# pixeli99/SVD_Xtend

Hardware: NVIDIA H100
Metric: SVD UNet train-step frames/sec @ 14x320x512 bf16 (higher is better)
Workload: dtype bf16

## Files before the change

### svd_xtend_b200/csrc/attention.cu

```cuda
#include "common.cuh"
#include "../../include/svd_xtend_b200.h"
#include "host_util.h"

namespace svdx {

constexpr int AT_THREADS = 288;
constexpr int AT_PRODUCER = 8;
constexpr int AT_CONSUMER_WARPS = 8;
constexpr int TILE_BYTES = 128 * 64 * 2;
constexpr float LOG2E = 1.4426950408889634f;

struct AttnKParams {
  CUtensorMap tq, tk, tv, tdo;
  int heads, S, G, RT, inner_groups, tiles, gshift, gmask;
  long long outer_stride, inner_stride, tok_stride;
  float scale;
  bf16* o; long long ldo;
  float* lse;
  float* delta;
  bf16* dq; long long lddq;
  bf16* dk; long long lddk;
  bf16* dv; long long lddv;
};

struct RowInfo {
  long long token;
  int g;
  bool valid;
};

SVDX_DEVINL RowInfo row_info(const AttnKParams& p, int r, int tile, int outer, int inner0) {
  RowInfo ri;
  const int t = tile * p.RT + (r >> p.gshift);
  ri.g = r & p.gmask;
  ri.valid = t < p.S;
  ri.token = (long long)outer * p.outer_stride + (long long)(inner0 + ri.g) * p.inner_stride + (long long)t * p.tok_stride;
  return ri;
}

SVDX_DEVINL float fast_exp2(float x) {
  float y;
  asm("ex2.approx.ftz.f32 %0, %1;" : "=f"(y) : "f"(x));
  return y;
}

SVDX_DEVINL void mma_abt64(float (&d)[32], uint32_t a_rows, uint32_t b_rows) {
  const uint64_t a = make_smem_desc_sw128(a_rows, 16, 1024), b = make_smem_desc_sw128(b_rows, 16, 1024);
  wgmma_fence();
#pragma unroll
  for (int ks = 0; ks < 4; ++ks) wgmma_ss_n64<0, 0>(d, a + 2 * ks, b + 2 * ks, ks > 0 ? 1u : 0u);
  wgmma_commit();
}
SVDX_DEVINL void mma_pb64(float (&acc)[32], const float (&p)[32], uint32_t b_rows) {
  const uint64_t b = make_smem_desc_sw128(b_rows, 8192, 1024);
  wgmma_fence();
#pragma unroll
  for (int ks = 0; ks < 4; ++ks)
    wgmma_rs_n64_tb(acc, pack_bf16x2(p[8 * ks], p[8 * ks + 1]), pack_bf16x2(p[8 * ks + 2], p[8 * ks + 3]),
                    pack_bf16x2(p[8 * ks + 4], p[8 * ks + 5]), pack_bf16x2(p[8 * ks + 6], p[8 * ks + 7]), b + (2048 >> 4) * ks, 1u);
  wgmma_commit();
}
SVDX_DEVINL int frag_col(int i, int lane) { return 8 * (i >> 2) + 2 * (lane & 3) + (i & 1); }
SVDX_DEVINL int frag_hi(int i) { return (i >> 1) & 1; }
SVDX_DEVINL float quad_max(float v) { return fmaxf(fmaxf(v, __shfl_xor_sync(0xffffffffu, v, 1)), __shfl_xor_sync(0xffffffffu, fmaxf(v, __shfl_xor_sync(0xffffffffu, v, 1)), 2)); }
SVDX_DEVINL float quad_sum(float v) { v += __shfl_xor_sync(0xffffffffu, v, 1); return v + __shfl_xor_sync(0xffffffffu, v, 2); }

SVDX_DEVINL void store_frag_rows(bf16* row_lo, bf16* row_hi, const float (&d)[32], float inv_lo, float inv_hi, int lane) {
#pragma unroll
  for (int j = 0; j < 8; ++j) {
    const int c = 8 * j + 2 * (lane & 3);
    if (row_lo) *reinterpret_cast<uint32_t*>(row_lo + c) = pack_bf16x2(d[4 * j] * inv_lo, d[4 * j + 1] * inv_lo);
    if (row_hi) *reinterpret_cast<uint32_t*>(row_hi + c) = pack_bf16x2(d[4 * j + 2] * inv_hi, d[4 * j + 3] * inv_hi);
  }
}

SVDX_DEVINL void decode_block(const AttnKParams& p, int& tile, int& head, int& outer, int& inner0) {
  tile = blockIdx.x;
  head = blockIdx.y;
  outer = blockIdx.z / p.inner_groups;
  inner0 = (blockIdx.z % p.inner_groups) * p.G;
}

SVDX_DEVINL void release(uint32_t bar, int lane) {
  __syncwarp();
  if (lane == 0) mbar_arrive(bar);
}

constexpr int FWD_KV_STAGES = 2;
constexpr int FWD_SMEM = 1024 + TILE_BYTES + FWD_KV_STAGES * 2 * TILE_BYTES + 256;

__global__ void __launch_bounds__(AT_THREADS, 1) attn_fwd_kernel(const __grid_constant__ AttnKParams p) {
  extern __shared__ uint8_t smem_raw[];
  const uint32_t base = (smem_u32(smem_raw) + 1023u) & ~1023u;
  const uint32_t sQ = base;
  const uint32_t sKV = sQ + TILE_BYTES;
  const uint32_t sBar = sKV + FWD_KV_STAGES * 2 * TILE_BYTES;
  const uint32_t b_qfull = sBar;
  const uint32_t b_kvfull = sBar + 8;
  const uint32_t b_kvempty = sBar + 8 * 3;

  const int warp = threadIdx.x >> 5, lane = threadIdx.x & 31;
  int tile, head, outer, inner0;
  decode_block(p, tile, head, outer, inner0);
  const int nkv = p.tiles;

  if (warp == AT_PRODUCER && lane == 0) {
    prefetch_tmap(&p.tq); prefetch_tmap(&p.tk); prefetch_tmap(&p.tv);
    mbar_init(b_qfull, 1);
    for (int i = 0; i < FWD_KV_STAGES; ++i) { mbar_init(b_kvfull + 8 * i, 1); mbar_init(b_kvempty + 8 * i, AT_CONSUMER_WARPS); }
    fence_barrier_init();
  }
  __syncthreads();

  if (warp == AT_PRODUCER) {
    if (lane == 0) {
      mbar_expect_tx(b_qfull, TILE_BYTES);
      tma_load_4d(&p.tq, b_qfull, sQ, head * 64, inner0, tile * p.RT, outer);
      for (int j = 0; j < nkv; ++j) {
        const int st = j % FWD_KV_STAGES;
        mbar_wait_mma(b_kvempty + 8 * st, ((j / FWD_KV_STAGES) & 1) ^ 1);
        mbar_expect_tx(b_kvfull + 8 * st, 2 * TILE_BYTES);
        tma_load_4d(&p.tk, b_kvfull + 8 * st, sKV + st * 2 * TILE_BYTES, head * 64, inner0, j * p.RT, outer);
        tma_load_4d(&p.tv, b_kvfull + 8 * st, sKV + st * 2 * TILE_BYTES + TILE_BYTES, head * 64, inner0, j * p.RT, outer);
      }
    }
    return;
  }
  const int wg = warp >> 2;
  const int r_lo = wg * 64 + (warp & 3) * 16 + (lane >> 2);
  const RowInfo ri[2] = {row_info(p, r_lo, tile, outer, inner0), row_info(p, r_lo + 8, tile, outer, inner0)};
  const float sc = p.scale * LOG2E;
  float m_run[2] = {-INFINITY, -INFINITY}, l_run[2] = {0.f, 0.f};
  float o[32];
#pragma unroll
  for (int i = 0; i < 32; ++i) o[i] = 0.f;
  mbar_wait_mma(b_qfull, 0);
  for (int j = 0; j < nkv; ++j) {
    const int st = j % FWD_KV_STAGES;
    const uint32_t sK = sKV + st * 2 * TILE_BYTES, sV = sK + TILE_BYTES;
    mbar_wait_mma(b_kvfull + 8 * st, (j / FWD_KV_STAGES) & 1);
    float s0[32], s1[32];
    mma_abt64(s0, sQ + wg * 8192, sK);
    mma_abt64(s1, sQ + wg * 8192, sK + 8192);
    wgmma_wait<0>();
    reg_fence(s0); reg_fence(s1);
    const int kvalid = p.S - j * p.RT;
    if (!(p.G == 1 && kvalid >= 128)) {
#pragma unroll
      for (int i = 0; i < 32; ++i) {
        const int c0 = frag_col(i, lane), c1 = 64 + c0;
        const RowInfo& r = ri[frag_hi(i)];
        if (!(((c0 & p.gmask) == r.g) && ((c0 >> p.gshift) < kvalid))) s0[i] = -INFINITY;
        if (!(((c1 & p.gmask) == r.g) && ((c1 >> p.gshift) < kvalid))) s1[i] = -INFINITY;
      }
    }
    float bm[2] = {-INFINITY, -INFINITY};
#pragma unroll
    for (int i = 0; i < 32; ++i) bm[frag_hi(i)] = fmaxf(bm[frag_hi(i)], fmaxf(s0[i], s1[i]));
    float msc[2], alpha[2];
#pragma unroll
    for (int h = 0; h < 2; ++h) {
      const float m_new = fmaxf(m_run[h], quad_max(bm[h]));
      const float m_use = m_new == -INFINITY ? 0.f : m_new;
      alpha[h] = fast_exp2((m_run[h] - m_use) * sc);
      m_run[h] = m_new;
      msc[h] = m_use * sc;
      l_run[h] *= alpha[h];
    }
#pragma unroll
    for (int i = 0; i < 32; ++i) {
      const int h = frag_hi(i);
      o[i] *= alpha[h];
      s0[i] = fast_exp2(fmaf(s0[i], sc, -msc[h]));
      s1[i] = fast_exp2(fmaf(s1[i], sc, -msc[h]));
      l_run[h] += s0[i] + s1[i];
    }
    mma_pb64(o, s0, sV);
    mma_pb64(o, s1, sV + 8192);
    wgmma_wait<0>();
    reg_fence(o);
    release(b_kvempty + 8 * st, lane);
  }
  bf16* rows[2];
  float inv[2];
#pragma unroll
  for (int h = 0; h < 2; ++h) {
    const float l = quad_sum(l_run[h]);
    const float m_use = m_run[h] == -INFINITY ? 0.f : m_run[h];
    inv[h] = 1.f / l;
    rows[h] = ri[h].valid ? p.o + ri[h].token * p.ldo + head * 64 : nullptr;
    if (ri[h].valid && p.lse && (lane & 3) == 0) p.lse[ri[h].token * p.heads + head] = m_use * p.scale + __logf(l);
  }
  store_frag_rows(rows[0], rows[1], o, inv[0], inv[1], lane);
}

constexpr int BWD_STAGES = 2;
constexpr int BDQ_SMEM = 1024 + 2 * TILE_BYTES + BWD_STAGES * 2 * TILE_BYTES + 256;

__global__ void __launch_bounds__(AT_THREADS, 1) attn_bwd_dq_kernel(const __grid_constant__ AttnKParams p) {
  extern __shared__ uint8_t smem_raw[];
  const uint32_t base = (smem_u32(smem_raw) + 1023u) & ~1023u;
  const uint32_t sQ = base, sDO = sQ + TILE_BYTES;
  const uint32_t sKV = sDO + TILE_BYTES;
  const uint32_t sBar = sKV + BWD_STAGES * 2 * TILE_BYTES;
  const uint32_t b_qfull = sBar;
  const uint32_t b_kvfull = sBar + 8;
  const uint32_t b_kvempty = sBar + 8 * 3;

  const int warp = threadIdx.x >> 5, lane = threadIdx.x & 31;
  int tile, head, outer, inner0;
  decode_block(p, tile, head, outer, inner0);
  const int nkv = p.tiles;

  if (warp == AT_PRODUCER && lane == 0) {
    prefetch_tmap(&p.tq); prefetch_tmap(&p.tk); prefetch_tmap(&p.tv); prefetch_tmap(&p.tdo);
    mbar_init(b_qfull, 1);
    for (int i = 0; i < BWD_STAGES; ++i) { mbar_init(b_kvfull + 8 * i, 1); mbar_init(b_kvempty + 8 * i, AT_CONSUMER_WARPS); }
    fence_barrier_init();
  }
  __syncthreads();

  if (warp == AT_PRODUCER) {
    if (lane == 0) {
      mbar_expect_tx(b_qfull, 2 * TILE_BYTES);
      tma_load_4d(&p.tq, b_qfull, sQ, head * 64, inner0, tile * p.RT, outer);
      tma_load_4d(&p.tdo, b_qfull, sDO, head * 64, inner0, tile * p.RT, outer);
      for (int j = 0; j < nkv; ++j) {
        const int st = j % BWD_STAGES;
        mbar_wait_mma(b_kvempty + 8 * st, ((j / BWD_STAGES) & 1) ^ 1);
        mbar_expect_tx(b_kvfull + 8 * st, 2 * TILE_BYTES);
        tma_load_4d(&p.tk, b_kvfull + 8 * st, sKV + st * 2 * TILE_BYTES, head * 64, inner0, j * p.RT, outer);
        tma_load_4d(&p.tv, b_kvfull + 8 * st, sKV + st * 2 * TILE_BYTES + TILE_BYTES, head * 64, inner0, j * p.RT, outer);
      }
    }
    return;
  }
  const int wg = warp >> 2;
  const int r_lo = wg * 64 + (warp & 3) * 16 + (lane >> 2);
  const RowInfo ri[2] = {row_info(p, r_lo, tile, outer, inner0), row_info(p, r_lo + 8, tile, outer, inner0)};
  const float sc = p.scale * LOG2E;
  float lse2[2], dlt[2];
#pragma unroll
  for (int h = 0; h < 2; ++h) {
    lse2[h] = ri[h].valid ? p.lse[ri[h].token * p.heads + head] * LOG2E : 0.f;
    dlt[h] = ri[h].valid ? p.delta[ri[h].token * p.heads + head] : 0.f;
  }
  float dq[32];
#pragma unroll
  for (int i = 0; i < 32; ++i) dq[i] = 0.f;
  mbar_wait_mma(b_qfull, 0);
  for (int j = 0; j < nkv; ++j) {
    const int st = j % BWD_STAGES;
    const uint32_t sK = sKV + st * 2 * TILE_BYTES, sV = sK + TILE_BYTES;
    mbar_wait_mma(b_kvfull + 8 * st, (j / BWD_STAGES) & 1);
    const int kvalid = p.S - j * p.RT;
    const bool nomask = (p.G == 1) && (kvalid >= 128);
#pragma unroll 1
    for (int kh = 0; kh < 2; ++kh) {
      float s[32], dp[32];
      mma_abt64(s, sQ + wg * 8192, sK + kh * 8192);
      mma_abt64(dp, sDO + wg * 8192, sV + kh * 8192);
      wgmma_wait<0>();
      reg_fence(s); reg_fence(dp);
#pragma unroll
      for (int i = 0; i < 32; ++i) {
        const int c = kh * 64 + frag_col(i, lane), h = frag_hi(i);
        const bool ok = ri[h].valid && (nomask || (((c & p.gmask) == ri[h].g) && ((c >> p.gshift) < kvalid)));
        const float pr = ok ? fast_exp2(fmaf(s[i], sc, -lse2[h])) * p.scale : 0.f;
        s[i] = pr * (dp[i] - dlt[h]);
      }
      mma_pb64(dq, s, sK + kh * 8192);
      wgmma_wait<0>();
      reg_fence(dq);
    }
    release(b_kvempty + 8 * st, lane);
  }
  store_frag_rows(ri[0].valid ? p.dq + ri[0].token * p.lddq + head * 64 : nullptr,
                  ri[1].valid ? p.dq + ri[1].token * p.lddq + head * 64 : nullptr, dq, 1.f, 1.f, lane);
}

constexpr int BKV_SMEM = 1024 + 2 * TILE_BYTES + BWD_STAGES * 2 * TILE_BYTES + 1024 + 256;

__global__ void __launch_bounds__(AT_THREADS, 1) attn_bwd_dkv_kernel(const __grid_constant__ AttnKParams p) {
  extern __shared__ uint8_t smem_raw[];
  const uint32_t base = (smem_u32(smem_raw) + 1023u) & ~1023u;
  const uint32_t sK = base, sV = sK + TILE_BYTES;
  const uint32_t sQD = sV + TILE_BYTES;
  const uint32_t sVec = sQD + BWD_STAGES * 2 * TILE_BYTES;
  const uint32_t sBar = sVec + 1024;
  const uint32_t b_kvfull = sBar;
  const uint32_t b_qfull = sBar + 8;
  const uint32_t b_qempty = sBar + 8 * 3;
  float* vec = reinterpret_cast<float*>(smem_raw + (sVec - smem_u32(smem_raw)));

  const int warp = threadIdx.x >> 5, lane = threadIdx.x & 31;
  int tile, head, outer, inner0;
  decode_block(p, tile, head, outer, inner0);
  const int nq = p.tiles;

  if (warp == AT_PRODUCER && lane == 0) {
    prefetch_tmap(&p.tq); prefetch_tmap(&p.tk); prefetch_tmap(&p.tv); prefetch_tmap(&p.tdo);
    mbar_init(b_kvfull, 1);
    for (int i = 0; i < BWD_STAGES; ++i) { mbar_init(b_qfull + 8 * i, 1); mbar_init(b_qempty + 8 * i, AT_CONSUMER_WARPS); }
    fence_barrier_init();
  }
  __syncthreads();

  if (warp == AT_PRODUCER) {
    if (lane == 0) {
      mbar_expect_tx(b_kvfull, 2 * TILE_BYTES);
      tma_load_4d(&p.tk, b_kvfull, sK, head * 64, inner0, tile * p.RT, outer);
      tma_load_4d(&p.tv, b_kvfull, sV, head * 64, inner0, tile * p.RT, outer);
      for (int i = 0; i < nq; ++i) {
        const int st = i % BWD_STAGES;
        mbar_wait_mma(b_qempty + 8 * st, ((i / BWD_STAGES) & 1) ^ 1);
        mbar_expect_tx(b_qfull + 8 * st, 2 * TILE_BYTES);
        tma_load_4d(&p.tq, b_qfull + 8 * st, sQD + st * 2 * TILE_BYTES, head * 64, inner0, i * p.RT, outer);
        tma_load_4d(&p.tdo, b_qfull + 8 * st, sQD + st * 2 * TILE_BYTES + TILE_BYTES, head * 64, inner0, i * p.RT, outer);
      }
    }
    return;
  }
  const int wg = warp >> 2;
  const int r_lo = wg * 64 + (warp & 3) * 16 + (lane >> 2);
  const RowInfo ki[2] = {row_info(p, r_lo, tile, outer, inner0), row_info(p, r_lo + 8, tile, outer, inner0)};
  const float sc = p.scale * LOG2E;
  const int vr = threadIdx.x & 127;
  auto load_stat = [&](int i) -> float {
    const RowInfo qi = row_info(p, vr, i, outer, inner0);
    if (threadIdx.x < 128) return qi.valid ? p.lse[qi.token * p.heads + head] * LOG2E : INFINITY;
    return qi.valid ? p.delta[qi.token * p.heads + head] : 0.f;
  };
  float stat = load_stat(0);
  float dv[32], dk[32];
#pragma unroll
  for (int i = 0; i < 32; ++i) { dv[i] = 0.f; dk[i] = 0.f; }
  mbar_wait_mma(b_kvfull, 0);
  for (int i = 0; i < nq; ++i) {
    named_bar_sync(1, 32 * AT_CONSUMER_WARPS);
    vec[threadIdx.x] = stat;
    named_bar_sync(1, 32 * AT_CONSUMER_WARPS);
    if (i + 1 < nq) stat = load_stat(i + 1);
    const int st = i % BWD_STAGES;
    const uint32_t sQ = sQD + st * 2 * TILE_BYTES, sDO = sQ + TILE_BYTES;
    mbar_wait_mma(b_qfull + 8 * st, (i / BWD_STAGES) & 1);
#pragma unroll 1
    for (int qh = 0; qh < 2; ++qh) {
      float s[32], dp[32];
      mma_abt64(s, sK + wg * 8192, sQ + qh * 8192);
      mma_abt64(dp, sV + wg * 8192, sDO + qh * 8192);
      wgmma_wait<0>();
      reg_fence(s); reg_fence(dp);
#pragma unroll
      for (int k = 0; k < 32; ++k) {
        const int c = qh * 64 + frag_col(k, lane);
        const RowInfo& r = ki[frag_hi(k)];
        const bool ok = r.valid && (p.G == 1 || (c & p.gmask) == r.g);
        const float pr = ok ? fast_exp2(fmaf(s[k], sc, -vec[c])) : 0.f;
        s[k] = pr;
        dp[k] = (pr * p.scale) * (dp[k] - vec[128 + c]);
      }
      mma_pb64(dv, s, sDO + qh * 8192);
      mma_pb64(dk, dp, sQ + qh * 8192);
      wgmma_wait<0>();
      reg_fence(dv); reg_fence(dk);
    }
    release(b_qempty + 8 * st, lane);
  }
  store_frag_rows(ki[0].valid ? p.dv + ki[0].token * p.lddv + head * 64 : nullptr,
                  ki[1].valid ? p.dv + ki[1].token * p.lddv + head * 64 : nullptr, dv, 1.f, 1.f, lane);
  store_frag_rows(ki[0].valid ? p.dk + ki[0].token * p.lddk + head * 64 : nullptr,
                  ki[1].valid ? p.dk + ki[1].token * p.lddk + head * 64 : nullptr, dk, 1.f, 1.f, lane);
}

__global__ void attn_delta_kernel(const bf16* __restrict__ o, long long ldo, const bf16* __restrict__ dout, long long lddo, long long tokens,
                                  int heads, float* __restrict__ delta) {
  const long long w = ((long long)blockIdx.x * blockDim.x + threadIdx.x) >> 5;
  const int lane = threadIdx.x & 31;
  if (w >= tokens * heads) return;
  const long long tok = w / heads;
  const int h = (int)(w - tok * heads);
  const float2 a = unpack_bf16x2(*reinterpret_cast<const uint32_t*>(o + tok * ldo + h * 64 + 2 * lane));
  const float2 b = unpack_bf16x2(*reinterpret_cast<const uint32_t*>(dout + tok * lddo + h * 64 + 2 * lane));
  const float s = warp_sum(a.x * b.x + a.y * b.y);
  if (lane == 0) delta[w] = s;
}

}

using namespace svdx;

static int attn_make_map(CUtensorMap* m, const void* ptr, int64_t ld, int cols, const SvdxAttn* d, int G, int RT) {
  const int outer = d->nseq / d->inner;
  uint64_t dims[4] = {(uint64_t)cols, (uint64_t)d->inner, (uint64_t)d->S, (uint64_t)outer};
  uint64_t strides[3] = {(uint64_t)(d->inner_stride * ld * 2), (uint64_t)(d->tok_stride * ld * 2), (uint64_t)(d->outer_stride * ld * 2)};
  if (d->inner == 1) strides[0] = (uint64_t)ld * 2;
  uint32_t box[4] = {64, (uint32_t)G, (uint32_t)RT, 1};
  return svdx_make_tmap(m, ptr, 4, dims, strides, box);
}

static int attn_setup(const SvdxAttn* d, AttnKParams& p, bool bwd, dim3& grid) {
  if (!d || !d->q || !d->k || !d->v) return svdx_fail(SVDX_E_BADARG, "attention: null pointer");
  if (d->heads <= 0 || d->S <= 0 || d->nseq <= 0 || d->inner <= 0 || d->nseq % d->inner) return svdx_fail(SVDX_E_BADARG, "attention: bad sequence geometry");
  if ((d->ldq % 8) || (d->ldk % 8) || (d->ldv % 8)) return svdx_fail(SVDX_E_BADARG, "attention: leading dims must be multiples of 8");
  memset(&p, 0, sizeof(p));
  int G = 1;
  if (d->inner > 1) {
    G = 1;
    while (G * 2 * d->S <= 128 && d->inner % (G * 2) == 0 && G < 64) G *= 2;
  }
  const int RT = 128 / G;
  if (d->inner > 1 && d->S > RT) return svdx_fail(SVDX_E_BADARG, "attention: strided sequences longer than 128 tokens are not supported");
  p.G = G; p.RT = RT; p.S = d->S; p.heads = d->heads;
  p.gmask = G - 1; p.gshift = 0;
  while ((1 << p.gshift) < G) ++p.gshift;
  p.inner_groups = d->inner / G;
  p.tiles = (d->S + RT - 1) / RT;
  p.outer_stride = d->outer_stride; p.inner_stride = d->inner_stride; p.tok_stride = d->tok_stride;
  p.scale = d->scale;
  const int cols = d->heads * 64;
  int rc;
  if ((rc = attn_make_map(&p.tq, d->q, d->ldq, cols, d, G, RT))) return rc;
  if ((rc = attn_make_map(&p.tk, d->k, d->ldk, cols, d, G, RT))) return rc;
  if ((rc = attn_make_map(&p.tv, d->v, d->ldv, cols, d, G, RT))) return rc;
  if (bwd) {
    if (!d->dout || !d->dq || !d->dk || !d->dv || !d->lse || !d->delta || !d->o) return svdx_fail(SVDX_E_BADARG, "attention_bwd: null pointer");
    if ((d->lddo % 8) || (d->lddq % 8) || (d->lddk % 8) || (d->lddv % 8) || (d->ldo % 8)) return svdx_fail(SVDX_E_BADARG, "attention_bwd: leading dims");
    if ((rc = attn_make_map(&p.tdo, d->dout, d->lddo, cols, d, G, RT))) return rc;
  } else {
    if (!d->o || (d->ldo % 8)) return svdx_fail(SVDX_E_BADARG, "attention_fwd: output");
  }
  p.o = reinterpret_cast<bf16*>(d->o); p.ldo = d->ldo;
  p.lse = d->lse; p.delta = d->delta;
  p.dq = reinterpret_cast<bf16*>(d->dq); p.lddq = d->lddq;
  p.dk = reinterpret_cast<bf16*>(d->dk); p.lddk = d->lddk;
  p.dv = reinterpret_cast<bf16*>(d->dv); p.lddv = d->lddv;
  const long long gz = (long long)(d->nseq / d->inner) * p.inner_groups;
  if (gz > 65535 || d->heads > 65535) return svdx_fail(SVDX_E_BADARG, "attention: grid too large");
  grid = dim3(p.tiles, d->heads, (unsigned)gz);
  return 0;
}

bool svdx_attention_small_eligible(const SvdxAttn* d);
int svdx_attention_small_fwd(const SvdxAttn* d, cudaStream_t st);
int svdx_attention_small_bwd(const SvdxAttn* d, cudaStream_t st);

extern "C" int svdx_attention_fwd(const SvdxAttn* d, void* stream_v) {
  cudaStream_t st = reinterpret_cast<cudaStream_t>(stream_v);
  if (svdx_attention_small_eligible(d)) return svdx_attention_small_fwd(d, st);
  AttnKParams p;
  dim3 grid;
// ... 6 lines not shown
    if (e != cudaSuccess) return svdx_fail_cuda(e, "attention_fwd: smem attribute");
    attr[slot] = true;
  }
  attn_fwd_kernel<<<grid, AT_THREADS, FWD_SMEM, st>>>(p);
  SVDX_CHECK_LAUNCH("attention_fwd");
  return SVDX_OK;
}

extern "C" int svdx_attention_bwd(const SvdxAttn* d, void* stream_v) {
  cudaStream_t st = reinterpret_cast<cudaStream_t>(stream_v);
  if (svdx_attention_small_eligible(d)) return svdx_attention_small_bwd(d, st);
  AttnKParams p;
  dim3 grid;
  int rc = attn_setup(d, p, true, grid);
  if (rc) return rc;
  static bool attr[SVDX_MAX_DEVICES] = {false};
  const int slot = svdx_device_slot();
  if (!attr[slot]) {
    cudaError_t e = cudaFuncSetAttribute(attn_bwd_dq_kernel, cudaFuncAttributeMaxDynamicSharedMemorySize, BDQ_SMEM);
    if (e == cudaSuccess) e = cudaFuncSetAttribute(attn_bwd_dkv_kernel, cudaFuncAttributeMaxDynamicSharedMemorySize, BKV_SMEM);
    if (e != cudaSuccess) return svdx_fail_cuda(e, "attention_bwd: smem attribute");
    attr[slot] = true;
  }
  const long long tokens = (long long)d->nseq * d->S;
  const long long warps = tokens * d->heads;
  attn_delta_kernel<<<(unsigned)((warps * 32 + 255) / 256), 256, 0, st>>>(reinterpret_cast<const bf16*>(d->o), d->ldo,
                                                                         reinterpret_cast<const bf16*>(d->dout), d->lddo, tokens, d->heads, d->delta);
  attn_bwd_dq_kernel<<<grid, AT_THREADS, BDQ_SMEM, st>>>(p);
  attn_bwd_dkv_kernel<<<grid, AT_THREADS, BKV_SMEM, st>>>(p);
  SVDX_CHECK_LAUNCH("attention_bwd");
  return SVDX_OK;
}
```

### svd_xtend_b200/csrc/common.cuh

```cuda
#pragma once
#include <cuda.h>
#include <cuda_bf16.h>
#include <cuda_runtime.h>
#include <stdint.h>
#include <stdio.h>

#include "wgmma.cuh"

namespace svdx {

typedef __nv_bfloat16 bf16;

#define SVDX_DEVINL __device__ __forceinline__

#ifndef SVDX_WAIT_TIMEOUT_CYCLES
#define SVDX_WAIT_TIMEOUT_CYCLES (4000000000ll)
#endif

SVDX_DEVINL uint32_t smem_u32(const void* p) { return (uint32_t)__cvta_generic_to_shared(p); }

SVDX_DEVINL uint32_t lane_id() { return threadIdx.x & 31; }

SVDX_DEVINL bool elect_one() {
  uint32_t pred = 0;
// ... 91 lines not shown
SVDX_DEVINL void tma_reduce_add_3d(const CUtensorMap* m, uint32_t src, int c0, int c1, int c2) {
  asm volatile("cp.reduce.async.bulk.tensor.3d.global.shared::cta.add.bulk_group [%0, {%2, %3, %4}], [%1];"
               ::"l"(reinterpret_cast<uint64_t>(m)), "r"(src), "r"(c0), "r"(c1), "r"(c2)
               : "memory");
}
SVDX_DEVINL void bulk_commit() { asm volatile("cp.async.bulk.commit_group;" ::: "memory"); }
template <int N>
SVDX_DEVINL void bulk_wait_read() { asm volatile("cp.async.bulk.wait_group.read %0;" ::"n"(N) : "memory"); }
template <int N>
SVDX_DEVINL void bulk_wait() { asm volatile("cp.async.bulk.wait_group %0;" ::"n"(N) : "memory"); }
SVDX_DEVINL void st_shared_v4(uint32_t addr, uint32_t a, uint32_t b, uint32_t c, uint32_t d) {
  asm volatile("st.shared.v4.b32 [%0], {%1, %2, %3, %4};" ::"r"(addr), "r"(a), "r"(b), "r"(c), "r"(d) : "memory");
}

SVDX_DEVINL void wgmma_fence() { asm volatile("wgmma.fence.sync.aligned;" ::: "memory"); }
SVDX_DEVINL void wgmma_commit() { asm volatile("wgmma.commit_group.sync.aligned;" ::: "memory"); }
template <int N>
SVDX_DEVINL void wgmma_wait() { asm volatile("wgmma.wait_group.sync.aligned %0;" ::"n"(N) : "memory"); }
template <int R>
SVDX_DEVINL void reg_fence(float (&d)[R]) {
#pragma unroll
  for (int i = 0; i < R; ++i) asm volatile("" : "+f"(d[i])::"memory");
}

SVDX_DEVINL void named_bar_sync(int id, int nthreads) { asm volatile("bar.sync %0, %1;" ::"r"(id), "r"(nthreads) : "memory"); }

SVDX_DEVINL uint64_t make_smem_desc_sw128(uint32_t saddr, uint32_t lbo_bytes, uint32_t sbo_bytes) {
  uint64_t d = 0;
  d |= (uint64_t)((saddr & 0x3FFFF) >> 4);
  d |= (uint64_t)((lbo_bytes >> 4) & 0x3FFF) << 16;
  d |= (uint64_t)((sbo_bytes >> 4) & 0x3FFF) << 32;
  d |= (uint64_t)1 << 62;
  return d;
}

SVDX_DEVINL float silu_f(float x) { return __fdividef(x, 1.0f + __expf(-x)); }
SVDX_DEVINL float silu_grad_f(float x) {
  const float s = __fdividef(1.0f, 1.0f + __expf(-x));
  return s * fmaf(x, 1.0f - s, 1.0f);
}
#define SVDX_HDINL __host__ __device__ __forceinline__
SVDX_HDINL float gelu_tail_log2(float ax) {
  float p = -1.92123457e-06f;
  p = fmaf(p, ax, 6.32884985e-05f);
  p = fmaf(p, ax, -0.000943420862f);
  p = fmaf(p, ax, 0.0085562719f);
  p = fmaf(p, ax, -0.0540522821f);
  p = fmaf(p, ax, -0.458381772f);
// ... 45 lines not shown
```

### svd_xtend_b200/raw.py

```python
from __future__ import annotations

import ctypes as C
import functools
import os
from typing import Optional, Sequence

import torch

from . import _lib
from ._lib import ACT_GELU, ACT_NONE, ACT_QUICK_GELU, A_CONV2D, A_ROWS, OUT_BF16, OUT_F32, OUT_F32_ATOMIC, SvdxAttn, SvdxTapGemm, load

bf16 = torch.bfloat16

_DTYPE_CODE = {torch.float32: 0, torch.bfloat16: 1, torch.float16: 2}


def dtype_code(t: torch.Tensor, what: str) -> int:
    try:
        return _DTYPE_CODE[t.dtype]
    except KeyError:
        raise TypeError(f"svd_xtend_b200: {what} has dtype {t.dtype}; supported: float32, bfloat16, float16") from None

LAUNCHES = [0]
_KERNELS_PER_CALL = {"svdx_groupnorm_apply_fused": 1, "svdx_attention_bwd": 3, "svdx_adamw_graph": 2, "svdx_adamw_p2p": 2,
                     "svdx_adamw_graph_ema": 2, "svdx_adamw_p2p_ema": 2, "svdx_ema_multi": 2, "svdx_adamw8bit": 2,
                     "svdx_adamw8bit_ema": 2}


def check(rc: int, what: str = "") -> None:
    LAUNCHES[0] += _KERNELS_PER_CALL.get(what, 1)
    _lib.check(rc, what)


ABLATE: set = set()
ACCOUNT = None
SHAPE_LOG = None


def _fam(family: str, flops: float = 0.0, nbytes: float = 0.0) -> bool:
    if ACCOUNT is not None:
        ACCOUNT(family, flops, nbytes)
    return family in ABLATE


def _stream() -> int:
    return torch.cuda.current_stream().cuda_stream

# ... 794 lines not shown
```

Before: 159.2.

## Software-pipeline attention kernels with ping-pong warpgroups, deeper stages, fused delta

The forward attention kernel now overlaps the next tile's QK^T wgmma with the previous tile's PV wgmma. It uses ping-pong named barriers so the two consumer warpgroups alternate tensor-core issue. The dq and dkv backward kernels are software-pipelined the same way by issuing the next half-tile's S/dP GEMMs while the current dS/P GEMMs run. Pipeline stages go from 2 to 4, and the separate delta kernel is folded into the dq kernel (the dkv producer reads lse/delta into per-stage smem). This costs more shared memory and register pressure, and adds an ordering dependency: the dkv kernel reads delta written by the dq kernel.

Result: faster. 161.3, median of 6 (+1.3%).

```diff
diff --git a/svd_xtend_b200/csrc/attention.cu b/svd_xtend_b200/csrc/attention.cu
--- a/svd_xtend_b200/csrc/attention.cu
+++ b/svd_xtend_b200/csrc/attention.cu
@@ -7,6 +7,7 @@
 constexpr int AT_THREADS = 288;
 constexpr int AT_PRODUCER = 8;
 constexpr int AT_CONSUMER_WARPS = 8;
+constexpr int AT_STAGES = 4;
 constexpr int TILE_BYTES = 128 * 64 * 2;
 constexpr float LOG2E = 1.4426950408889634f;
 
@@ -16,6 +17,7 @@
   long long outer_stride, inner_stride, tok_stride;
   float scale;
   bf16* o; long long ldo;
+  const bf16* dout; long long lddo;
   float* lse;
   float* delta;
   bf16* dq; long long lddq;
@@ -44,21 +46,33 @@
   return y;
 }
 
-SVDX_DEVINL void mma_abt64(float (&d)[32], uint32_t a_rows, uint32_t b_rows) {
+SVDX_DEVINL void mma_abt128(float (&d)[64], uint32_t a_rows, uint32_t b_rows) {
   const uint64_t a = make_smem_desc_sw128(a_rows, 16, 1024), b = make_smem_desc_sw128(b_rows, 16, 1024);
   wgmma_fence();
 #pragma unroll
-  for (int ks = 0; ks < 4; ++ks) wgmma_ss_n64<0, 0>(d, a + 2 * ks, b + 2 * ks, ks > 0 ? 1u : 0u);
+  for (int ks = 0; ks < 4; ++ks) wgmma_ss_n128<0, 0>(d, a + 2 * ks, b + 2 * ks, ks > 0 ? 1u : 0u);
   wgmma_commit();
 }
-SVDX_DEVINL void mma_pb64(float (&acc)[32], const float (&p)[32], uint32_t b_rows) {
+SVDX_DEVINL void mma_abt64x2(float (&s)[32], uint32_t a1, uint32_t b1, float (&dp)[32], uint32_t a2, uint32_t b2) {
+  const uint64_t da1 = make_smem_desc_sw128(a1, 16, 1024), db1 = make_smem_desc_sw128(b1, 16, 1024);
+  const uint64_t da2 = make_smem_desc_sw128(a2, 16, 1024), db2 = make_smem_desc_sw128(b2, 16, 1024);
+  wgmma_fence();
+#pragma unroll
+  for (int ks = 0; ks < 4; ++ks) wgmma_ss_n64<0, 0>(s, da1 + 2 * ks, db1 + 2 * ks, ks > 0 ? 1u : 0u);
+#pragma unroll
+  for (int ks = 0; ks < 4; ++ks) wgmma_ss_n64<0, 0>(dp, da2 + 2 * ks, db2 + 2 * ks, ks > 0 ? 1u : 0u);
+  wgmma_commit();
+}
+template <int KS>
+SVDX_DEVINL void mma_rb(float (&acc)[32], const uint32_t (&a)[4 * KS], uint32_t b_rows) {
   const uint64_t b = make_smem_desc_sw128(b_rows, 8192, 1024);
-  wgmma_fence();
-#pragma unroll
-  for (int ks = 0; ks < 4; ++ks)
-    wgmma_rs_n64_tb(acc, pack_bf16x2(p[8 * ks], p[8 * ks + 1]), pack_bf16x2(p[8 * ks + 2], p[8 * ks + 3]),
-                    pack_bf16x2(p[8 * ks + 4], p[8 * ks + 5]), pack_bf16x2(p[8 * ks + 6], p[8 * ks + 7]), b + (2048 >> 4) * ks, 1u);
-  wgmma_commit();
+#pragma unroll
+  for (int ks = 0; ks < KS; ++ks) wgmma_rs_n64_tb(acc, a[4 * ks], a[4 * ks + 1], a[4 * ks + 2], a[4 * ks + 3], b + (2048 >> 4) * ks, 1u);
+}
+template <int R>
+SVDX_DEVINL void pack_frag(uint32_t (&a)[R / 2], const float (&d)[R]) {
+#pragma unroll
+  for (int i = 0; i < R / 2; ++i) a[i] = pack_bf16x2(d[2 * i], d[2 * i + 1]);
 }
 SVDX_DEVINL int frag_col(int i, int lane) { return 8 * (i >> 2) + 2 * (lane & 3) + (i & 1); }
 SVDX_DEVINL int frag_hi(int i) { return (i >> 1) & 1; }
@@ -86,18 +100,56 @@
   if (lane == 0) mbar_arrive(bar);
 }
 
-constexpr int FWD_KV_STAGES = 2;
-constexpr int FWD_SMEM = 1024 + TILE_BYTES + FWD_KV_STAGES * 2 * TILE_BYTES + 256;
+struct PingPong {
+  int wg;
+  SVDX_DEVINL void start() const { if (wg == 1) named_bar_arrive(1, 32 * AT_CONSUMER_WARPS); }
+  SVDX_DEVINL void acquire() const { named_bar_sync(1 + wg, 32 * AT_CONSUMER_WARPS); }
+  SVDX_DEVINL void pass(bool last) const { if (wg == 0 || !last) named_bar_arrive(2 - wg, 32 * AT_CONSUMER_WARPS); }
+};
+
+constexpr int FWD_SMEM = 1024 + TILE_BYTES + AT_STAGES * 2 * TILE_BYTES + 256;
+
+SVDX_DEVINL void online_softmax(const AttnKParams& p, float (&s)[64], float (&m_run)[2], float (&l_run)[2], float (&alpha)[2],
+                                const RowInfo (&ri)[2], int kvalid, float sc, int lane) {
+  if (!(p.G == 1 && kvalid >= 128)) {
+#pragma unroll
+    for (int i = 0; i < 64; ++i) {
+      const int c = frag_col(i, lane);
+      const RowInfo& r = ri[frag_hi(i)];
+      if (!(((c & p.gmask) == r.g) && ((c >> p.gshift) < kvalid))) s[i] = -INFINITY;
+    }
+  }
+  float bm[2] = {-INFINITY, -INFINITY};
+#pragma unroll
+  for (int i = 0; i < 32; ++i) bm[frag_hi(i)] = fmaxf(bm[frag_hi(i)], fmaxf(s[i], s[i + 32]));
+  float msc[2];
+#pragma unroll
+  for (int h = 0; h < 2; ++h) {
+    const float m_new = fmaxf(m_run[h], quad_max(bm[h]));
+    const float m_use = m_new == -INFINITY ? 0.f : m_new;
+    alpha[h] = fast_exp2((m_run[h] - m_use) * sc);
+    m_run[h] = m_new;
+    msc[h] = m_use * sc;
+    l_run[h] *= alpha[h];
+  }
+#pragma unroll
+  for (int i = 0; i < 32; ++i) {
+    const int h = frag_hi(i);
+    s[i] = fast_exp2(fmaf(s[i], sc, -msc[h]));
+    s[i + 32] = fast_exp2(fmaf(s[i + 32], sc, -msc[h]));
+    l_run[h] += s[i] + s[i + 32];
+  }
+}
 
 __global__ void __launch_bounds__(AT_THREADS, 1) attn_fwd_kernel(const __grid_constant__ AttnKParams p) {
   extern __shared__ uint8_t smem_raw[];
   const uint32_t base = (smem_u32(smem_raw) + 1023u) & ~1023u;
   const uint32_t sQ = base;
   const uint32_t sKV = sQ + TILE_BYTES;
-  const uint32_t sBar = sKV + FWD_KV_STAGES * 2 * TILE_BYTES;
+  const uint32_t sBar = sKV + AT_STAGES * 2 * TILE_BYTES;
   const uint32_t b_qfull = sBar;
   const uint32_t b_kvfull = sBar + 8;
-  const uint32_t b_kvempty = sBar + 8 * 3;
+  const uint32_t b_kvempty = sBar + 8 * (1 + AT_STAGES);
 
   const int warp = threadIdx.x >> 5, lane = threadIdx.x & 31;
   int tile, head, outer, inner0;
@@ -107,7 +159,7 @@
   if (warp == AT_PRODUCER && lane == 0) {
     prefetch_tmap(&p.tq); prefetch_tmap(&p.tk); prefetch_tmap(&p.tv);
     mbar_init(b_qfull, 1);
-    for (int i = 0; i < FWD_KV_STAGES; ++i) { mbar_init(b_kvfull + 8 * i, 1); mbar_init(b_kvempty + 8 * i, AT_CONSUMER_WARPS); }
+    for (int i = 0; i < AT_STAGES; ++i) { mbar_init(b_kvfull + 8 * i, 1); mbar_init(b_kvempty + 8 * i, AT_CONSUMER_WARPS); }
     fence_barrier_init();
   }
   __syncthreads();
@@ -117,8 +169,8 @@
       mbar_expect_tx(b_qfull, TILE_BYTES);
       tma_load_4d(&p.tq, b_qfull, sQ, head * 64, inner0, tile * p.RT, outer);
       for (int j = 0; j < nkv; ++j) {
-        const int st = j % FWD_KV_STAGES;
-        mbar_wait_mma(b_kvempty + 8 * st, ((j / FWD_KV_STAGES) & 1) ^ 1);
+        const int st = j % AT_STAGES;
+        mbar_wait_mma(b_kvempty + 8 * st, ((j / AT_STAGES) & 1) ^ 1);
         mbar_expect_tx(b_kvfull + 8 * st, 2 * TILE_BYTES);
         tma_load_4d(&p.tk, b_kvfull + 8 * st, sKV + st * 2 * TILE_BYTES, head * 64, inner0, j * p.RT, outer);
         tma_load_4d(&p.tv, b_kvfull + 8 * st, sKV + st * 2 * TILE_BYTES + TILE_BYTES, head * 64, inner0, j * p.RT, outer);
@@ -130,57 +182,49 @@
   const int r_lo = wg * 64 + (warp & 3) * 16 + (lane >> 2);
   const RowInfo ri[2] = {row_info(p, r_lo, tile, outer, inner0), row_info(p, r_lo + 8, tile, outer, inner0)};
   const float sc = p.scale * LOG2E;
-  float m_run[2] = {-INFINITY, -INFINITY}, l_run[2] = {0.f, 0.f};
-  float o[32];
+  const uint32_t sQw = sQ + wg * 8192;
+  const PingPong pp{wg};
+  float m_run[2] = {-INFINITY, -INFINITY}, l_run[2] = {0.f, 0.f}, alpha[2];
+  float o[32], s[64];
+  uint32_t pa[32];
 #pragma unroll
   for (int i = 0; i < 32; ++i) o[i] = 0.f;
+  pp.start();
   mbar_wait_mma(b_qfull, 0);
-  for (int j = 0; j < nkv; ++j) {
-    const int st = j % FWD_KV_STAGES;
-    const uint32_t sK = sKV + st * 2 * TILE_BYTES, sV = sK + TILE_BYTES;
-    mbar_wait_mma(b_kvfull + 8 * st, (j / FWD_KV_STAGES) & 1);
-    float s0[32], s1[32];
-    mma_abt64(s0, sQ + wg * 8192, sK);
-    mma_abt64(s1, sQ + wg * 8192, sK + 8192);
+  mbar_wait_mma(b_kvfull, 0);
+  pp.acquire();
+  mma_abt128(s, sQw, sKV);
+  pp.pass(false);
+  wgmma_wait<0>();
+  reg_fence(s);
+  online_softmax(p, s, m_run, l_run, alpha, ri, p.S, sc, lane);
+  pack_frag<64>(pa, s);
+  for (int j = 1; j < nkv; ++j) {
+    const int st = j % AT_STAGES, pst = (j - 1) % AT_STAGES;
+    mbar_wait_mma(b_kvfull + 8 * st, (j / AT_STAGES) & 1);
+    pp.acquire();
+    mma_abt128(s, sQw, sKV + st * 2 * TILE_BYTES);
+    wgmma_fence();
+    mma_rb<8>(o, pa, sKV + pst * 2 * TILE_BYTES + TILE_BYTES);
+    wgmma_commit();
+    pp.pass(false);
+    wgmma_wait<1>();
+    reg_fence(s);
+    online_softmax(p, s, m_run, l_run, alpha, ri, p.S - j * p.RT, sc, lane);
     wgmma_wait<0>();
-    reg_fence(s0); reg_fence(s1);
-    const int kvalid = p.S - j * p.RT;
-    if (!(p.G == 1 && kvalid >= 128)) {
-#pragma unroll
-      for (int i = 0; i < 32; ++i) {
-        const int c0 = frag_col(i, lane), c1 = 64 + c0;
-        const RowInfo& r = ri[frag_hi(i)];
-        if (!(((c0 & p.gmask) == r.g) && ((c0 >> p.gshift) < kvalid))) s0[i] = -INFINITY;
-        if (!(((c1 & p.gmask) == r.g) && ((c1 >> p.gshift) < kvalid))) s1[i] = -INFINITY;
-      }
-    }
-    float bm[2] = {-INFINITY, -INFINITY};
-#pragma unroll
-    for (int i = 0; i < 32; ++i) bm[frag_hi(i)] = fmaxf(bm[frag_hi(i)], fmaxf(s0[i], s1[i]));
-    float msc[2], alpha[2];
-#pragma unroll
-    for (int h = 0; h < 2; ++h) {
-      const float m_new = fmaxf(m_run[h], quad_max(bm[h]));
-      const float m_use = m_new == -INFINITY ? 0.f : m_new;
-      alpha[h] = fast_exp2((m_run[h] - m_use) * sc);
-      m_run[h] = m_new;
-      msc[h] = m_use * sc;
-      l_run[h] *= alpha[h];
-    }
-#pragma unroll
-    for (int i = 0; i < 32; ++i) {
-      const int h = frag_hi(i);
-      o[i] *= alpha[h];
-      s0[i] = fast_exp2(fmaf(s0[i], sc, -msc[h]));
-      s1[i] = fast_exp2(fmaf(s1[i], sc, -msc[h]));
-      l_run[h] += s0[i] + s1[i];
-    }
-    mma_pb64(o, s0, sV);
-    mma_pb64(o, s1, sV + 8192);
-    wgmma_wait<0>();
-    reg_fence(o);
-    release(b_kvempty + 8 * st, lane);
-  }
+    reg_fence(o); reg_fence(pa);
+    release(b_kvempty + 8 * pst, lane);
+#pragma unroll
+    for (int i = 0; i < 32; ++i) o[i] *= alpha[frag_hi(i)];
+    pack_frag<64>(pa, s);
+  }
+  pp.acquire();
+  wgmma_fence();
+  mma_rb<8>(o, pa, sKV + ((nkv - 1) % AT_STAGES) * 2 * TILE_BYTES + TILE_BYTES);
+  wgmma_commit();
+  pp.pass(true);
+  wgmma_wait<0>();
+  reg_fence(o);
   bf16* rows[2];
   float inv[2];
 #pragma unroll
@@ -194,18 +238,35 @@
   store_frag_rows(rows[0], rows[1], o, inv[0], inv[1], lane);
 }
 
-constexpr int BWD_STAGES = 2;
-constexpr int BDQ_SMEM = 1024 + 2 * TILE_BYTES + BWD_STAGES * 2 * TILE_BYTES + 256;
+constexpr int BDQ_SMEM = 1024 + 2 * TILE_BYTES + AT_STAGES * 2 * TILE_BYTES + 256;
+
+SVDX_DEVINL float row_delta(const bf16* o, const bf16* dout, bool valid, int lane) {
+  const int q = lane & 3;
+  float t[8];
+#pragma unroll
+  for (int m = 0; m < 8; ++m) {
+    float2 a = make_float2(0.f, 0.f), b = a;
+    if (valid) {
+      a = unpack_bf16x2(*reinterpret_cast<const uint32_t*>(o + 2 * (q + 4 * m)));
+      b = unpack_bf16x2(*reinterpret_cast<const uint32_t*>(dout + 2 * (q + 4 * m)));
+    }
+    t[m] = fmaf(a.x, b.x, a.y * b.y);
+  }
+  const float w0 = t[0] + t[4], w1 = t[1] + t[5], w2 = t[2] + t[6], w3 = t[3] + t[7];
+  float v = (w0 + w2) + (w1 + w3);
+  v += __shfl_xor_sync(0xffffffffu, v, 2);
+  return v + __shfl_xor_sync(0xffffffffu, v, 1);
+}
 
 __global__ void __launch_bounds__(AT_THREADS, 1) attn_bwd_dq_kernel(const __grid_constant__ AttnKParams p) {
   extern __shared__ uint8_t smem_raw[];
   const uint32_t base = (smem_u32(smem_raw) + 1023u) & ~1023u;
   const uint32_t sQ = base, sDO = sQ + TILE_BYTES;
   const uint32_t sKV = sDO + TILE_BYTES;
-  const uint32_t sBar = sKV + BWD_STAGES * 2 * TILE_BYTES;
+  const uint32_t sBar = sKV + AT_STAGES * 2 * TILE_BYTES;
   const uint32_t b_qfull = sBar;
   const uint32_t b_kvfull = sBar + 8;
-  const uint32_t b_kvempty = sBar + 8 * 3;
+  const uint32_t b_kvempty = sBar + 8 * (1 + AT_STAGES);
 
   const int warp = threadIdx.x >> 5, lane = threadIdx.x & 31;
   int tile, head, outer, inner0;
@@ -215,7 +276,7 @@
   if (warp == AT_PRODUCER && lane == 0) {
     prefetch_tmap(&p.tq); prefetch_tmap(&p.tk); prefetch_tmap(&p.tv); prefetch_tmap(&p.tdo);
     mbar_init(b_qfull, 1);
-    for (int i = 0; i < BWD_STAGES; ++i) { mbar_init(b_kvfull + 8 * i, 1); mbar_init(b_kvempty + 8 * i, AT_CONSUMER_WARPS); }
+    for (int i = 0; i < AT_STAGES; ++i) { mbar_init(b_kvfull + 8 * i, 1); mbar_init(b_kvempty + 8 * i, AT_CONSUMER_WARPS); }
     fence_barrier_init();
   }
   __syncthreads();
@@ -226,8 +287,8 @@
       tma_load_4d(&p.tq, b_qfull, sQ, head * 64, inner0, tile * p.RT, outer);
       tma_load_4d(&p.tdo, b_qfull, sDO, head * 64, inner0, tile * p.RT, outer);
       for (int j = 0; j < nkv; ++j) {
-        const int st = j % BWD_STAGES;
-        mbar_wait_mma(b_kvempty + 8 * st, ((j / BWD_STAGES) & 1) ^ 1);
+        const int st = j % AT_STAGES;
+        mbar_wait_mma(b_kvempty + 8 * st, ((j / AT_STAGES) & 1) ^ 1);
         mbar_expect_tx(b_kvfull + 8 * st, 2 * TILE_BYTES);
         tma_load_4d(&p.tk, b_kvfull + 8 * st, sKV + st * 2 * TILE_BYTES, head * 64, inner0, j * p.RT, outer);
         tma_load_4d(&p.tv, b_kvfull + 8 * st, sKV + st * 2 * TILE_BYTES + TILE_BYTES, head * 64, inner0, j * p.RT, outer);
@@ -243,54 +304,68 @@
 #pragma unroll
   for (int h = 0; h < 2; ++h) {
     lse2[h] = ri[h].valid ? p.lse[ri[h].token * p.heads + head] * LOG2E : 0.f;
-    dlt[h] = ri[h].valid ? p.delta[ri[h].token * p.heads + head] : 0.f;
-  }
-  float dq[32];
+    dlt[h] = row_delta(p.o + ri[h].token * p.ldo + head * 64, p.dout + ri[h].token * p.lddo + head * 64, ri[h].valid, lane);
+    if (ri[h].valid && (lane & 3) == 0) p.delta[ri[h].token * p.heads + head] = dlt[h];
+  }
+  const uint32_t sQw = sQ + wg * 8192, sDOw = sDO + wg * 8192;
+  float dq[32], s[32], dp[32];
+  uint32_t ds[16];
 #pragma unroll
   for (int i = 0; i < 32; ++i) dq[i] = 0.f;
+  reg_fence(dq);
+  const int nu = 2 * nkv;
   mbar_wait_mma(b_qfull, 0);
-  for (int j = 0; j < nkv; ++j) {
-    const int st = j % BWD_STAGES;
-    const uint32_t sK = sKV + st * 2 * TILE_BYTES, sV = sK + TILE_BYTES;
-    mbar_wait_mma(b_kvfull + 8 * st, (j / BWD_STAGES) & 1);
+  mbar_wait_mma(b_kvfull, 0);
+  mma_abt64x2(s, sQw, sKV, dp, sDOw, sKV + TILE_BYTES);
+  for (int u = 0; u < nu; ++u) {
+    const int j = u >> 1, kh = u & 1, st = j % AT_STAGES;
+    const uint32_t sK = sKV + st * 2 * TILE_BYTES;
+    wgmma_wait<0>();
+    reg_fence(s); reg_fence(dp); reg_fence(dq); reg_fence(ds);
+    if (u >= 2 && kh == 0) release(b_kvempty + 8 * ((j - 1) % AT_STAGES), lane);
     const int kvalid = p.S - j * p.RT;
     const bool nomask = (p.G == 1) && (kvalid >= 128);
-#pragma unroll 1
-    for (int kh = 0; kh < 2; ++kh) {
-      float s[32], dp[32];
-      mma_abt64(s, sQ + wg * 8192, sK + kh * 8192);
-      mma_abt64(dp, sDO + wg * 8192, sV + kh * 8192);
-      wgmma_wait<0>();
-      reg_fence(s); reg_fence(dp);
-#pragma unroll
-      for (int i = 0; i < 32; ++i) {
-        const int c = kh * 64 + frag_col(i, lane), h = frag_hi(i);
+#pragma unroll
+    for (int i = 0; i < 32; i += 2) {
+      float v[2];
+#pragma unroll
+      for (int e = 0; e < 2; ++e) {
+        const int c = kh * 64 + frag_col(i + e, lane), h = frag_hi(i + e);
         const bool ok = ri[h].valid && (nomask || (((c & p.gmask) == ri[h].g) && ((c >> p.gshift) < kvalid)));
-        const float pr = ok ? fast_exp2(fmaf(s[i], sc, -lse2[h])) * p.scale : 0.f;
-        s[i] = pr * (dp[i] - dlt[h]);
+        const float pr = ok ? fast_exp2(fmaf(s[i + e], sc, -lse2[h])) * p.scale : 0.f;
+        v[e] = pr * (dp[i + e] - dlt[h]);
       }
-      mma_pb64(dq, s, sK + kh * 8192);
-      wgmma_wait<0>();
-      reg_fence(dq);
-    }
-    release(b_kvempty + 8 * st, lane);
-  }
+      ds[i / 2] = pack_bf16x2(v[0], v[1]);
+    }
+    const bool more = u + 1 < nu;
+    const int j1 = (u + 1) >> 1, st1 = j1 % AT_STAGES;
+    if (more && kh == 1) mbar_wait_mma(b_kvfull + 8 * st1, (j1 / AT_STAGES) & 1);
+    wgmma_fence();
+    mma_rb<4>(dq, ds, sK + kh * 8192);
+    wgmma_commit();
+    if (more) {
+      const uint32_t sK1 = sKV + st1 * 2 * TILE_BYTES, c1 = ((u + 1) & 1) * 8192;
+      mma_abt64x2(s, sQw, sK1 + c1, dp, sDOw, sK1 + TILE_BYTES + c1);
+    }
+  }
+  wgmma_wait<0>();
+  reg_fence(dq);
   store_frag_rows(ri[0].valid ? p.dq + ri[0].token * p.lddq + head * 64 : nullptr,
                   ri[1].valid ? p.dq + ri[1].token * p.lddq + head * 64 : nullptr, dq, 1.f, 1.f, lane);
 }
 
-constexpr int BKV_SMEM = 1024 + 2 * TILE_BYTES + BWD_STAGES * 2 * TILE_BYTES + 1024 + 256;
+constexpr int BKV_SMEM = 1024 + 2 * TILE_BYTES + AT_STAGES * 2 * TILE_BYTES + AT_STAGES * 1024 + 256;
 
 __global__ void __launch_bounds__(AT_THREADS, 1) attn_bwd_dkv_kernel(const __grid_constant__ AttnKParams p) {
   extern __shared__ uint8_t smem_raw[];
   const uint32_t base = (smem_u32(smem_raw) + 1023u) & ~1023u;
   const uint32_t sK = base, sV = sK + TILE_BYTES;
   const uint32_t sQD = sV + TILE_BYTES;
-  const uint32_t sVec = sQD + BWD_STAGES * 2 * TILE_BYTES;
-  const uint32_t sBar = sVec + 1024;
+  const uint32_t sVec = sQD + AT_STAGES * 2 * TILE_BYTES;
+  const uint32_t sBar = sVec + AT_STAGES * 1024;
   const uint32_t b_kvfull = sBar;
   const uint32_t b_qfull = sBar + 8;
-  const uint32_t b_qempty = sBar + 8 * 3;
+  const uint32_t b_qempty = sBar + 8 * (1 + AT_STAGES);
   float* vec = reinterpret_cast<float*>(smem_raw + (sVec - smem_u32(smem_raw)));
 
   const int warp = threadIdx.x >> 5, lane = threadIdx.x & 31;
@@ -301,89 +376,102 @@
   if (warp == AT_PRODUCER && lane == 0) {
     prefetch_tmap(&p.tq); prefetch_tmap(&p.tk); prefetch_tmap(&p.tv); prefetch_tmap(&p.tdo);
     mbar_init(b_kvfull, 1);
-    for (int i = 0; i < BWD_STAGES; ++i) { mbar_init(b_qfull + 8 * i, 1); mbar_init(b_qempty + 8 * i, AT_CONSUMER_WARPS); }
+    for (int i = 0; i < AT_STAGES; ++i) { mbar_init(b_qfull + 8 * i, 1 + 32); mbar_init(b_qempty + 8 * i, AT_CONSUMER_WARPS); }
     fence_barrier_init();
   }
   __syncthreads();
 
   if (warp == AT_PRODUCER) {
-    if (lane == 0) {
-      mbar_expect_tx(b_kvfull, 2 * TILE_BYTES);
-      tma_load_4d(&p.tk, b_kvfull, sK, head * 64, inner0, tile * p.RT, outer);
-      tma_load_4d(&p.tv, b_kvfull, sV, head * 64, inner0, tile * p.RT, outer);
+    {
+      if (lane == 0) {
+        mbar_expect_tx(b_kvfull, 2 * TILE_BYTES);
+        tma_load_4d(&p.tk, b_kvfull, sK, head * 64, inner0, tile * p.RT, outer);
+        tma_load_4d(&p.tv, b_kvfull, sV, head * 64, inner0, tile * p.RT, outer);
+      }
       for (int i = 0; i < nq; ++i) {
-        const int st = i % BWD_STAGES;
-        mbar_wait_mma(b_qempty + 8 * st, ((i / BWD_STAGES) & 1) ^ 1);
-        mbar_expect_tx(b_qfull + 8 * st, 2 * TILE_BYTES);
-        tma_load_4d(&p.tq, b_qfull + 8 * st, sQD + st * 2 * TILE_BYTES, head * 64, inner0, i * p.RT, outer);
-        tma_load_4d(&p.tdo, b_qfull + 8 * st, sQD + st * 2 * TILE_BYTES + TILE_BYTES, head * 64, inner0, i * p.RT, outer);
+        const int st = i % AT_STAGES;
+        mbar_wait_mma(b_qempty + 8 * st, ((i / AT_STAGES) & 1) ^ 1);
+        if (lane == 0) {
+          mbar_expect_tx(b_qfull + 8 * st, 2 * TILE_BYTES);
+          tma_load_4d(&p.tq, b_qfull + 8 * st, sQD + st * 2 * TILE_BYTES, head * 64, inner0, i * p.RT, outer);
+          tma_load_4d(&p.tdo, b_qfull + 8 * st, sQD + st * 2 * TILE_BYTES + TILE_BYTES, head * 64, inner0, i * p.RT, outer);
+        }
+#pragma unroll
+        for (int k = 0; k < 4; ++k) {
+          const int r = lane + 32 * k;
+          const RowInfo qi = row_info(p, r, i, outer, inner0);
+          vec[st * 256 + r] = qi.valid ? p.lse[qi.token * p.heads + head] * LOG2E : INFINITY;
+          vec[st * 256 + 128 + r] = qi.valid ? p.delta[qi.token * p.heads + head] : 0.f;
+        }
+        mbar_arrive(b_qfull + 8 * st);
       }
     }
     return;
   }
   const int wg = warp >> 2;
   const int r_lo = wg * 64 + (warp & 3) * 16 + (lane >> 2);
+  bool kval[2];
+  int kg[2];
+#pragma unroll
+  for (int h = 0; h < 2; ++h) {
+    const RowInfo r = row_info(p, r_lo + 8 * h, tile, outer, inner0);
+    kval[h] = r.valid;
+    kg[h] = r.g;
+  }
+  const float sc = p.scale * LOG2E;
+  const uint32_t sKw = sK + wg * 8192, sVw = sV + wg * 8192;
+  float dv[32], dk[32], s[32], dp[32];
+  uint32_t pt[16], dst[16];
+#pragma unroll
+  for (int i = 0; i < 32; ++i) { dv[i] = 0.f; dk[i] = 0.f; }
+  reg_fence(dv); reg_fence(dk);
+  const int nu = 2 * nq;
+  mbar_wait_mma(b_kvfull, 0);
+  mbar_wait_mma(b_qfull, 0);
+  mma_abt64x2(s, sKw, sQD, dp, sVw, sQD + TILE_BYTES);
+  for (int u = 0; u < nu; ++u) {
+    const int i = u >> 1, qh = u & 1, st = i % AT_STAGES;
+    const uint32_t sQ = sQD + st * 2 * TILE_BYTES, sDO = sQ + TILE_BYTES;
+    const float* lse2 = vec + st * 256 + qh * 64 + 2 * (lane & 3);
+    const float* dlt = lse2 + 128;
+    wgmma_wait<0>();
+    reg_fence(s); reg_fence(dp); reg_fence(dv); reg_fence(dk); reg_fence(pt); reg_fence(dst);
+    if (u >= 2 && qh == 0) release(b_qempty + 8 * ((i - 1) % AT_STAGES), lane);
+#pragma unroll
+    for (int k = 0; k < 32; k += 2) {
+      const float2 l2 = *reinterpret_cast<const float2*>(lse2 + 8 * (k >> 2));
+      const float2 d2 = *reinterpret_cast<const float2*>(dlt + 8 * (k >> 2));
+      float pr[2], ds[2];
+#pragma unroll
+      for (int e = 0; e < 2; ++e) {
+        const int c = qh * 64 + frag_col(k + e, lane);
+        const int h = frag_hi(k + e);
+        const bool ok = kval[h] && (p.G == 1 || (c & p.gmask) == kg[h]);
+        pr[e] = ok ? fast_exp2(fmaf(s[k + e], sc, -(e ? l2.y : l2.x))) : 0.f;
+        ds[e] = (pr[e] * p.scale) * (dp[k + e] - (e ? d2.y : d2.x));
+      }
+      pt[k / 2] = pack_bf16x2(pr[0], pr[1]);
+      dst[k / 2] = pack_bf16x2(ds[0], ds[1]);
+    }
+    const bool more = u + 1 < nu;
+    const int i1 = (u + 1) >> 1, st1 = i1 % AT_STAGES;
+    if (more && qh == 1) mbar_wait_mma(b_qfull + 8 * st1, (i1 / AT_STAGES) & 1);
+    wgmma_fence();
+    mma_rb<4>(dv, pt, sDO + qh * 8192);
+    mma_rb<4>(dk, dst, sQ + qh * 8192);
+    wgmma_commit();
+    if (more) {
+      const uint32_t sQ1 = sQD + st1 * 2 * TILE_BYTES, c1 = ((u + 1) & 1) * 8192;
+      mma_abt64x2(s, sKw, sQ1 + c1, dp, sVw, sQ1 + TILE_BYTES + c1);
+    }
+  }
+  wgmma_wait<0>();
+  reg_fence(dv); reg_fence(dk);
   const RowInfo ki[2] = {row_info(p, r_lo, tile, outer, inner0), row_info(p, r_lo + 8, tile, outer, inner0)};
-  const float sc = p.scale * LOG2E;
-  const int vr = threadIdx.x & 127;
-  auto load_stat = [&](int i) -> float {
-    const RowInfo qi = row_info(p, vr, i, outer, inner0);
-    if (threadIdx.x < 128) return qi.valid ? p.lse[qi.token * p.heads + head] * LOG2E : INFINITY;
-    return qi.valid ? p.delta[qi.token * p.heads + head] : 0.f;
-  };
-  float stat = load_stat(0);
-  float dv[32], dk[32];
-#pragma unroll
-  for (int i = 0; i < 32; ++i) { dv[i] = 0.f; dk[i] = 0.f; }
-  mbar_wait_mma(b_kvfull, 0);
-  for (int i = 0; i < nq; ++i) {
-    named_bar_sync(1, 32 * AT_CONSUMER_WARPS);
-    vec[threadIdx.x] = stat;
-    named_bar_sync(1, 32 * AT_CONSUMER_WARPS);
-    if (i + 1 < nq) stat = load_stat(i + 1);
-    const int st = i % BWD_STAGES;
-    const uint32_t sQ = sQD + st * 2 * TILE_BYTES, sDO = sQ + TILE_BYTES;
-    mbar_wait_mma(b_qfull + 8 * st, (i / BWD_STAGES) & 1);
-#pragma unroll 1
-    for (int qh = 0; qh < 2; ++qh) {
-      float s[32], dp[32];
-      mma_abt64(s, sK + wg * 8192, sQ + qh * 8192);
-      mma_abt64(dp, sV + wg * 8192, sDO + qh * 8192);
-      wgmma_wait<0>();
-      reg_fence(s); reg_fence(dp);
-#pragma unroll
-      for (int k = 0; k < 32; ++k) {
-        const int c = qh * 64 + frag_col(k, lane);
-        const RowInfo& r = ki[frag_hi(k)];
-        const bool ok = r.valid && (p.G == 1 || (c & p.gmask) == r.g);
-        const float pr = ok ? fast_exp2(fmaf(s[k], sc, -vec[c])) : 0.f;
-        s[k] = pr;
-        dp[k] = (pr * p.scale) * (dp[k] - vec[128 + c]);
-      }
-      mma_pb64(dv, s, sDO + qh * 8192);
-      mma_pb64(dk, dp, sQ + qh * 8192);
-      wgmma_wait<0>();
-      reg_fence(dv); reg_fence(dk);
-    }
-    release(b_qempty + 8 * st, lane);
-  }
   store_frag_rows(ki[0].valid ? p.dv + ki[0].token * p.lddv + head * 64 : nullptr,
                   ki[1].valid ? p.dv + ki[1].token * p.lddv + head * 64 : nullptr, dv, 1.f, 1.f, lane);
   store_frag_rows(ki[0].valid ? p.dk + ki[0].token * p.lddk + head * 64 : nullptr,
                   ki[1].valid ? p.dk + ki[1].token * p.lddk + head * 64 : nullptr, dk, 1.f, 1.f, lane);
-}
-
-__global__ void attn_delta_kernel(const bf16* __restrict__ o, long long ldo, const bf16* __restrict__ dout, long long lddo, long long tokens,
-                                  int heads, float* __restrict__ delta) {
-  const long long w = ((long long)blockIdx.x * blockDim.x + threadIdx.x) >> 5;
-  const int lane = threadIdx.x & 31;
-  if (w >= tokens * heads) return;
-  const long long tok = w / heads;
-  const int h = (int)(w - tok * heads);
-  const float2 a = unpack_bf16x2(*reinterpret_cast<const uint32_t*>(o + tok * ldo + h * 64 + 2 * lane));
-  const float2 b = unpack_bf16x2(*reinterpret_cast<const uint32_t*>(dout + tok * lddo + h * 64 + 2 * lane));
-  const float s = warp_sum(a.x * b.x + a.y * b.y);
-  if (lane == 0) delta[w] = s;
 }
 
 }
@@ -427,6 +515,7 @@
     if (!d->dout || !d->dq || !d->dk || !d->dv || !d->lse || !d->delta || !d->o) return svdx_fail(SVDX_E_BADARG, "attention_bwd: null pointer");
     if ((d->lddo % 8) || (d->lddq % 8) || (d->lddk % 8) || (d->lddv % 8) || (d->ldo % 8)) return svdx_fail(SVDX_E_BADARG, "attention_bwd: leading dims");
     if ((rc = attn_make_map(&p.tdo, d->dout, d->lddo, cols, d, G, RT))) return rc;
+    p.dout = reinterpret_cast<const bf16*>(d->dout); p.lddo = d->lddo;
   } else {
     if (!d->o || (d->ldo % 8)) return svdx_fail(SVDX_E_BADARG, "attention_fwd: output");
   }
@@ -479,10 +568,6 @@
     if (e != cudaSuccess) return svdx_fail_cuda(e, "attention_bwd: smem attribute");
     attr[slot] = true;
   }
-  const long long tokens = (long long)d->nseq * d->S;
-  const long long warps = tokens * d->heads;
-  attn_delta_kernel<<<(unsigned)((warps * 32 + 255) / 256), 256, 0, st>>>(reinterpret_cast<const bf16*>(d->o), d->ldo,
-                                                                         reinterpret_cast<const bf16*>(d->dout), d->lddo, tokens, d->heads, d->delta);
   attn_bwd_dq_kernel<<<grid, AT_THREADS, BDQ_SMEM, st>>>(p);
   attn_bwd_dkv_kernel<<<grid, AT_THREADS, BKV_SMEM, st>>>(p);
   SVDX_CHECK_LAUNCH("attention_bwd");
diff --git a/svd_xtend_b200/csrc/common.cuh b/svd_xtend_b200/csrc/common.cuh
--- a/svd_xtend_b200/csrc/common.cuh
+++ b/svd_xtend_b200/csrc/common.cuh
@@ -137,8 +137,14 @@
 #pragma unroll
   for (int i = 0; i < R; ++i) asm volatile("" : "+f"(d[i])::"memory");
 }
+template <int R>
+SVDX_DEVINL void reg_fence(uint32_t (&d)[R]) {
+#pragma unroll
+  for (int i = 0; i < R; ++i) asm volatile("" : "+r"(d[i])::"memory");
+}
 
 SVDX_DEVINL void named_bar_sync(int id, int nthreads) { asm volatile("bar.sync %0, %1;" ::"r"(id), "r"(nthreads) : "memory"); }
+SVDX_DEVINL void named_bar_arrive(int id, int nthreads) { asm volatile("bar.arrive %0, %1;" ::"r"(id), "r"(nthreads) : "memory"); }
 
 SVDX_DEVINL uint64_t make_smem_desc_sw128(uint32_t saddr, uint32_t lbo_bytes, uint32_t sbo_bytes) {
   uint64_t d = 0;
diff --git a/svd_xtend_b200/raw.py b/svd_xtend_b200/raw.py
--- a/svd_xtend_b200/raw.py
+++ b/svd_xtend_b200/raw.py
@@ -22,7 +22,7 @@
         raise TypeError(f"svd_xtend_b200: {what} has dtype {t.dtype}; supported: float32, bfloat16, float16") from None
 
 LAUNCHES = [0]
-_KERNELS_PER_CALL = {"svdx_groupnorm_apply_fused": 1, "svdx_attention_bwd": 3, "svdx_adamw_graph": 2, "svdx_adamw_p2p": 2,
+_KERNELS_PER_CALL = {"svdx_groupnorm_apply_fused": 1, "svdx_attention_bwd": 2, "svdx_adamw_graph": 2, "svdx_adamw_p2p": 2,
                      "svdx_adamw_graph_ema": 2, "svdx_adamw_p2p_ema": 2, "svdx_ema_multi": 2, "svdx_adamw8bit": 2,
                      "svdx_adamw8bit_ema": 2}
 
```
